# zhangyu2ustc/GCN_fmri_decoding

Hardware: AMD Instinct MI355X
Metric: fMRI-windows/sec (fwd+bwd) 6-layer ChebNet K=5 N≈10k; HBM GB/s vs roofline (higher is better)
Workload: dtype f32; 1 GPU; BASELINE configs[1]: ChebNet K=5 x6 conv (F=32, p=1, b2relu), FC 512-256-22, synthetic N=10000 kNN-8 graph -> M=10466, block_dura=15, batch 64 per GPU; global_batch=64, parallelism=dp1, step=fwd+loss+bwd+allreduce+Adam, batch gathered on device

## Files before the change

gcn_fmri_decoding_amd/_lib.py:

```python
import ctypes as C
import os

_HERE = os.path.dirname(os.path.abspath(__file__))
LIB_PATH = os.environ.get('CHEBGCN_LIB') or os.path.join(_HERE, 'libchebgcn.so')

BIAS_NONE, BIAS_FILTER, BIAS_VERTEX = 0, 1, 2
POOL_MAX, POOL_AVG = 0, 1
KNN_EUCLIDEAN, KNN_COSINE, KNN_CORRELATION, KNN_DOT = 0, 1, 2, 3
KNN_KMAX = 32
MC_SITES = 16
PARCEL_MEAN, PARCEL_SUM = 0, 1


class ChebgcnError(RuntimeError):
    pass


_p = C.c_void_p
_i = C.c_int
_i64 = C.c_int64
_f = C.c_float

SIGNATURES = {
    'chebgcn_version': (_i, []),
# ... 33 lines not shown
    'chebgcn_brelu_pool_bwd_workspace': (C.c_size_t, [_i, _i, _i, _i, _i]),
    'chebgcn_brelu_pool_bwd': (_i, [_p, _p, _p, _p, _p, _i, _i, _i, _i, _i, _i, _i, _p, C.c_size_t, _p]),
    'chebgcn_pool_gather_fwd': (_i, [_p, _p, _p, _p, _i, _i, _i, _i, _i, _i, _p]),
    'chebgcn_pool_scatter_bwd_workspace': (C.c_size_t, [_i, _i, _i, _i, _i]),
    'chebgcn_pool_scatter_bwd': (_i, [_p, _p, _p, _p, _p, _i, _i, _i, _i, _i, _i, _i, _p, C.c_size_t, _p]),
    'chebgcn_contract_bwd_w_workspace': (C.c_size_t, [_i, _i, _i, _i, _i]),
    'chebgcn_contract_bwd_w': (_i, [_p, _p, _p, _p, C.c_size_t, _i, _i, _i, _i, _i, _p]),
    'chebgcn_contract_bwd_x': (_i, [_p, _p, _p, _i, _i, _i, _i, _i, _p]),
    'chebgcn_contract_bwd_x_relu': (_i, [_p, _p, _p, _p, _i, _i, _i, _i, _i, _p]),
    'chebgcn_contract_bwd_w_relu': (_i, [_p, _p, _p, _p, _p, C.c_size_t, _i, _i, _i, _i, _i, _p]),
    'chebgcn_contract_bwd_w_relu_bias_merged': (_i, [_i, _i, _i, _i, _i]),
    'chebgcn_contract_bwd_w_relu_bias': (_i, [_p, _p, _p, _p, _p, _p, C.c_size_t, _i, _i, _i, _i, _i, _p]),
    'chebgcn_contract_fwd_mean_supported': (_i, [_i, _i, _i, _i, _i]),
    'chebgcn_contract_fwd_gated_supported': (_i, [_i, _i, _i, _i, _i]),
    'chebgcn_contract_fwd_gated': (_i, [_p, _p, _p, _p, _i, _i, _i, _i, _i, _p]),
    'chebgcn_contract_fwd_mean': (_i, [_p, _p, _p, _i, _p, _p, _i, _i, _i, _i, _i, _p]),
    'chebgcn_contract_bwd_w_relu_mean': (_i, [_p, _p, _p, _p, _p, C.c_size_t, _i, _i, _i, _i, _i, _p]),
    'chebgcn_contract_bwd_x_relu_mean': (_i, [_p, _p, _p, _p, _i, _i, _i, _i, _i, _p]),
    'chebgcn_bias_grad_relu_mean': (_i, [_p, _p, _p, _i, _i, _i, _i, _p, C.c_size_t, _p]),
    'chebgcn_relu_grad_mean': (_i, [_p, _p, _p, _p, _i, _i, _i, _i, _p, C.c_size_t, _p]),
    'chebgcn_fused_layer_supported': (_i, [_p, _i, _i, _i, _i]),
    'chebgcn_fused_layer_workspace': (C.c_size_t, [_p, _i, _i, _i, _i]),
    'chebgcn_fused_layer_fwd': (_i, [_p, _p, _p, _p, _i, _p, _p, _p, _p, C.c_size_t, _i, _i, _i, _i, _i, _p]),
    'chebgcn_fused_layer_bwd_x': (_i, [_p, _p, _p, _p, _p, _i, _i, _i, _i, _p]),
    'chebgcn_perm_data': (_i, [_p, _p, _p, _p, _i, _i, _i, _i, _p]),
    'chebgcn_to_plane': (_i, [_p, _p, _i, _i, _i, _p]),
    'chebgcn_from_plane': (_i, [_p, _p, _i, _i, _i, _p]),
    'chebgcn_feature_mean_fwd': (_i, [_p, _p, _i, _i, _i, _p]),
    'chebgcn_feature_mean_bwd': (_i, [_p, _p, _i, _i, _i, _p]),
    'chebgcn_fc_fwd_supported': (_i, [_i, _i, _i]),
    'chebgcn_fc_fwd_workspace': (C.c_size_t, [_i, _i, _i]),
    'chebgcn_fc_fwd': (_i, [_p, _i64, _p, _p, _p, _p, C.c_size_t, _i, _i, _i, _i, _p]),
    'chebgcn_fc_bwd': (_i, [_p, _i64, _p, _p, _p, _p, _p, _p, _i64, _i, _i, _i, _p]),
    'chebgcn_planes_to_rows': (_i, [_p, _p, _p, _i, _i, _i, _i64, _p]),
    'chebgcn_rows_to_planes': (_i, [_p, _p, _p, _i, _i, _i, _i64, _p]),
    'chebgcn_adam_step': (_i, [_p, _p, _p, _p, _i64, _f, _f, _f, _f, _f, _f, _p]),
    'chebgcn_adam_step_dev': (_i, [_p, _p, _p, _p, _i64, _p, _f, _f, _f, _f, _f, _p]),
    'chebgcn_metis_one_level_f32': (_i, [_i64, _p, _p, _p, _p, _p, _i64, _p]),
    'chebgcn_metis_one_level_f32p': (_i, [_i64, _p, _p, _p, _p, _p, _i64, _p]),
    'chebgcn_metis_one_level_f64': (_i, [_i64, _p, _p, _p, _p, _p, _i64, _p]),
    'chebgcn_compute_perm_level': (_i, [_p, _i64, _p, _i64, _p]),
    'chebgcn_bank_order': (_i, [_i, _p, _p, _i, _p, _p]),
    'chebgcn_spectral_transform': (_i, [_p, _p, _p, _i, _i, _i, _p]),
    'chebgcn_spectral_mix_fwd': (_i, [_p, _p, _p, _i, _i, _i, _i, _p]),
    'chebgcn_spectral_mix_bwd_x': (_i, [_p, _p, _p, _i, _i, _i, _i, _p]),
    'chebgcn_spectral_mix_bwd_w': (_i, [_p, _p, _p, _i, _i, _i, _i, _p]),
    'chebgcn_spectral_spline_expand': (_i, [_p, _p, _p, _i, _i, _i, _p]),
    'chebgcn_spectral_spline_expand_bwd': (_i, [_p, _p, _p, _i, _i, _i, _p]),
    'chebgcn_saliency_supported': (_i, [_i]),
    'chebgcn_saliency_seed': (_i, [_p, _p, _i, _i, _i, _p, _p, _i, _i, _p]),
    'chebgcn_saliency_path': (_i, [_p, _p, _p, _p, _p, _i, _i, _i, _i, _i, _i, _p]),
    'chebgcn_saliency_reduce': (_i, [_p, _p, _p, _p, _p, _i, _i, _i, _i, _i, _i, _p, _p, _i, _p, _p]),
    'chebgcn_occlusion_supported': (_i, [_i]),
    'chebgcn_occlusion_rows': (_i, [_p, _p, _p, _p, _p, _i64, _i, _i, _i, _i, _i, _i, _p]),
    'chebgcn_occlusion_score': (_i, [_p, _i64, _i, _i, _i, _i, _p, _i, _p, _p, _p]),
    'chebgcn_occlusion_class_sums': (_i, [_p, _p, _i, _i, _i, _p, _p]),
    'chebgcn_shapley_supported': (_i, [_i]),
    'chebgcn_shapley_rows': (_i, [_p, _p, _p, _p, _p, _p, _i64, _i, _i, _i, _i, _i, _i, _i, _p]),
    'chebgcn_shapley_score': (_i, [_p, _i64, _i, _i, _i, _i, _i, _p, _i, _p, _p]),
    'chebgcn_shapley_reduce': (_i, [_p, _p, _i, _i, _i, _p, _p]),
    'chebgcn_gradcam_weights': (_i, [_p, _i, _i, _i, _p, _p]),
    'chebgcn_gradcam_map': (_i, [_p, _p, _p, _p, _i, _i, _i, _i, _i, _p, _i64, _p]),
    'chebgcn_gather_windows': (_i, [_p, _i64, _p, _p, _p, _p, _p, _i, _i, _i, _p]),
    'chebgcn_gather_windows_mix': (_i, [_p, _i64, _p, _p, _i, _p, _p, _p, _p, _i, _i, _i, _p]),
    'chebgcn_window_stats_workspace': (C.c_size_t, [_i64, _i, _i]),
    'chebgcn_window_stats': (_i, [_p, _i64, _p, _i64, _p, _p, _p, _p, _i, _i, _p, C.c_size_t, _p]),
# ... 59 lines not shown
```

gcn_fmri_decoding_amd/csrc/head.hip:

```cpp
#include <hip/hip_runtime.h>
#include "../../include/chebgcn.h"
#include "status.h"
#include "contract_common.h"
#include "aug_draw.h"

namespace chebgcn {

constexpr int FC_WAVES = 8;
constexpr int FC_CHUNK = 32;
constexpr int FC_U = 2;

__global__ void __launch_bounds__(FC_WAVES * 64)
fc_fwd_kernel(const float* __restrict__ x, long long ldx, const float* __restrict__ W, const float* __restrict__ bias,
              float* __restrict__ y, float* __restrict__ part_out, int B, int I, int O, int relu, int cps) {
    __shared__ float part[FC_WAVES][32][33];
    const int lane = threadIdx.x & 63, wave = threadIdx.x >> 6;
    const int c = lane & 31, h = lane >> 5;
    const int bx = blockIdx.x, by = blockIdx.y, bz = blockIdx.z;
    const int o0 = bx * 32, b0 = by * 32;
    const int brow = min(b0 + c, B - 1), ocol = min(o0 + c, O - 1);
    const float* xr = x + (size_t)brow * ldx;
    const float* wc = W + ocol;
    const int nchunks = (I + FC_CHUNK - 1) / FC_CHUNK;
    const int q_lo = bz * cps, q_hi = min(q_lo + cps, nchunks);
    f32x16 acc;
#pragma unroll
    for (int j = 0; j < 16; ++j) acc[j] = 0.f;
    for (int q0 = q_lo + wave; q0 < q_hi; q0 += FC_WAVES * FC_U) {
        f32x4 av[FC_U][4];
        float bv[FC_U][4][4];
#pragma unroll
        for (int u = 0; u < FC_U; ++u) {
            const int q = q0 + FC_WAVES * u;
            const int k = (q < q_hi ? FC_CHUNK * q : 0) + 16 * h;
#pragma unroll
            for (int t = 0; t < 4; ++t) {
                av[u][t] = *reinterpret_cast<const f32x4*>(xr + (k + 4 * t + 3 < ldx ? k + 4 * t : 0));
// ... 328 lines not shown
        }
        const float et = expf(row[t] - m);
        acc += et > 1e-30f ? log1pf(so / et) : logf(s) - (row[t] - m);
        const float inv = invB / s;
        for (int c = 0; c < C; ++c) drow[c] = c == t ? -so * inv : expf(row[c] - m) * inv;
    }
    part[threadIdx.x] = acc;
    __syncthreads();
    for (int d = 128; d > 0; d >>= 1) {
        if ((int)threadIdx.x < d) part[threadIdx.x] += part[threadIdx.x + d];
        __syncthreads();
    }
    if (threadIdx.x == 0) *loss = part[0] * invB;
}
}

using namespace chebgcn;

static int fc_splits(int B, int I, int O) {
    const int tiles = ((O + 31) / 32) * ((B + 31) / 32);
    int s = 512 / tiles;
    const int by_len = (I + 511) / 512;
    if (s > by_len) s = by_len;
    return s < 1 ? 1 : s;
}

extern "C" int chebgcn_fc_fwd_supported(int B, int I, int O) {
    return B > 0 && I > 0 && O > 0 && I <= (1 << 20) && (long long)B * O <= (1 << 20);
}

extern "C" size_t chebgcn_fc_fwd_workspace(int B, int I, int O) {
    if (!chebgcn_fc_fwd_supported(B, I, O)) return 0;
    const int S = fc_splits(B, I, O);
    return S > 1 ? (size_t)S * B * O * sizeof(float) : 0;
}

extern "C" int chebgcn_fc_fwd(const float* x, int64_t ldx, const float* W, const float* bias, float* y, void* workspace,
                              size_t workspace_bytes, int B, int I, int O, int relu, chebgcn_stream stream_) {
    hipStream_t stream = (hipStream_t)stream_;
    CG_REQUIRE(x && W && y && B > 0 && I > 0 && O > 0 && ldx >= I, "fc_fwd: bad argument");
    if (!chebgcn_fc_fwd_supported(B, I, O) || (ldx & 3) || ((uintptr_t)x & 15))
        return CHEBGCN_EUNSUPPORTED;
    const int S = fc_splits(B, I, O);
    const int nchunks = (I + FC_CHUNK - 1) / FC_CHUNK, cps = (nchunks + S - 1) / S;
    CG_REQUIRE(S == 1 || (workspace && workspace_bytes >= chebgcn_fc_fwd_workspace(B, I, O)), "fc_fwd: workspace too small");
    dim3 grid((O + 31) / 32, (B + 31) / 32, S);
    note_dispatch(S > 1 ? "fc_fwd_kernel<split>" : "fc_fwd_kernel");
    if (S > 1) note_dispatch_more("fc_fwd_reduce_kernel");
    hipLaunchKernelGGL(fc_fwd_kernel, grid, dim3(FC_WAVES * 64), 0, stream, x, (long long)ldx, W, bias, y,
                       S > 1 ? (float*)workspace : nullptr, B, I, O, relu, cps);
    if (S > 1)
        hipLaunchKernelGGL(fc_fwd_reduce_kernel, dim3((B * O + 255) / 256), dim3(256), 0, stream, (const float*)workspace, bias,
                           y, B * O, O, S, relu);
    CG_HIP(hipGetLastError());
    return CHEBGCN_OK;
}

static int fc_dropout_splits(int S, int B, int I, int O) {
    const long long tiles = (long long)S * ((O + 31) / 32) * ((B + 31) / 32);
    long long s = 512 / tiles;
    const int by_len = (I + 511) / 512;
    if (s > by_len) s = by_len;
    return s < 1 ? 1 : (int)s;
}

extern "C" int chebgcn_fc_fwd_dropout_supported(int S, int B, int I, int O) {
    return S > 0 && S <= 32768 && B > 0 && I > 0 && O > 0 && I <= (1 << 20) && (long long)S * B * O <= (1 << 20);
}

extern "C" size_t chebgcn_fc_fwd_dropout_workspace(int S, int B, int I, int O) {
    if (!chebgcn_fc_fwd_dropout_supported(S, B, I, O)) return 0;
    const int ns = fc_dropout_splits(S, B, I, O);
    return ns > 1 ? (size_t)ns * S * B * O * sizeof(float) : 0;
}

// ... 5 lines not shown
    CG_REQUIRE(x && W && y && win && S > 0 && B > 0 && I > 0 && O > 0 && ldx >= I, "fc_fwd_dropout: bad argument");
    CG_REQUIRE(sample_stride == 0 || sample_stride >= (int64_t)(B - 1) * ldx + I,
               "fc_fwd_dropout: a sample stride of %lld elements is neither 0 nor a whole [B][ldx] matrix", (long long)sample_stride);
    CG_REQUIRE(s0 >= 0 && layer >= 0 && layer < CHEBGCN_MC_SITES, "fc_fwd_dropout: bad sample number %d or dropout site %d", s0,
               layer);
    CG_REQUIRE(inv_keep >= 1.f && inv_keep < __builtin_inff(), "fc_fwd_dropout: inv_keep = 1 / keep must be a finite number >= 1");
    if (!chebgcn_fc_fwd_dropout_supported(S, B, I, O) || (ldx & 3) || (sample_stride & 3) || ((uintptr_t)x & 15))
        return CHEBGCN_EUNSUPPORTED;
    const int ns = fc_dropout_splits(S, B, I, O);
    const int nchunks = (I + FC_CHUNK - 1) / FC_CHUNK, cps = (nchunks + ns - 1) / ns;
    CG_REQUIRE(ns == 1 || (workspace && workspace_bytes >= chebgcn_fc_fwd_dropout_workspace(S, B, I, O)),
               "fc_fwd_dropout: workspace too small");
    dim3 grid((O + 31) / 32, (B + 31) / 32, S * ns);
    if (sample_stride == 0)
        note_dispatch(ns > 1 ? "fc_fwd_dropout_kernel<shared, split>" : "fc_fwd_dropout_kernel<shared>");
    else
        note_dispatch(ns > 1 ? "fc_fwd_dropout_kernel<per_sample, split>" : "fc_fwd_dropout_kernel<per_sample>");
    if (ns > 1) note_dispatch_more("fc_fwd_reduce_kernel");
    hipLaunchKernelGGL(fc_fwd_dropout_kernel, grid, dim3(FC_WAVES * 64), 0, stream, x, (long long)ldx, (long long)sample_stride, W,
                       bias, y, ns > 1 ? (float*)workspace : nullptr, win, S, B, I, O, relu, cps, ns, seed, (uint32_t)s0,
                       (uint32_t)layer, threshold, inv_keep);
    if (ns > 1)
        hipLaunchKernelGGL(fc_fwd_reduce_kernel, dim3((S * B * O + 255) / 256), dim3(256), 0, stream, (const float*)workspace,
                           bias, y, S * B * O, O, ns, relu);
    CG_HIP(hipGetLastError());
    return CHEBGCN_OK;
}

extern "C" int chebgcn_fc_bwd(const float* x, int64_t ldx, const float* W, const float* g, const float* y, float* dW,
                              float* db, float* dx, int64_t lddx, int B, int I, int O, chebgcn_stream stream_) {
    hipStream_t stream = (hipStream_t)stream_;
    CG_REQUIRE(x && W && g && B > 0 && I > 0 && O > 0 && ldx >= I && (!dx || lddx >= I), "fc_bwd: bad argument");
    if (!chebgcn_fc_fwd_supported(B, I, O)) return CHEBGCN_EUNSUPPORTED;
    note_dispatch(dW ? "fc_bwd_w_kernel" : "");
    if (dW) {
        dim3 grid((O + 31) / 32, (I + 31) / 32);
        hipLaunchKernelGGL(fc_bwd_w_kernel, grid, dim3(FC_WAVES * 64), 0, stream, x, (long long)ldx, g, y, dW, db, B, I, O);
    }
    if (dx) {
        dim3 grid((I + 31) / 32, (B + 31) / 32);
        const bool vec = (O & 3) == 0 && ((uintptr_t)g & 15) == 0 && ((uintptr_t)W & 15) == 0 && (!y || ((uintptr_t)y & 15) == 0);
        note_dispatch_more(vec ? "fc_bwd_x_kernel<true>" : "fc_bwd_x_kernel<false>");
        if (vec)
            hipLaunchKernelGGL(fc_bwd_x_kernel<true>, grid, dim3(FC_WAVES * 64), 0, stream, g, y, W, dx, (long long)lddx, B, I, O);
        else
            hipLaunchKernelGGL(fc_bwd_x_kernel<false>, grid, dim3(FC_WAVES * 64), 0, stream, g, y, W, dx, (long long)lddx, B, I, O);
    }
    CG_HIP(hipGetLastError());
    return CHEBGCN_OK;
}

static int planes_rows(bool to_rows, const float* src, float* dst, const int32_t* order, int B, int M, int F, int64_t ldr,
                       hipStream_t stream) {
    CG_REQUIRE(src && dst && B > 0 && B <= 65535 && M > 0 && F > 0 && ldr >= (int64_t)M * F,
               to_rows ? "planes_to_rows: bad argument" : "rows_to_planes: bad argument");
    const int Mp = plane_stride(M);
    dim3 grid(((to_rows ? M : Mp) + FLAT_V - 1) / FLAT_V, B);
    note_dispatch(to_rows ? "planes_rows_kernel<to_rows>" : "planes_rows_kernel<to_planes>");
    if (to_rows)
        hipLaunchKernelGGL(planes_rows_kernel<true>, grid, dim3(256), 0, stream, src, dst, order, M, Mp, F, (long long)ldr);
    else
        hipLaunchKernelGGL(planes_rows_kernel<false>, grid, dim3(256), 0, stream, src, dst, order, M, Mp, F, (long long)ldr);
    CG_HIP(hipGetLastError());
    return CHEBGCN_OK;
}

extern "C" int chebgcn_planes_to_rows(const float* planes, float* rows, const int32_t* order, int B, int M, int F, int64_t ldr,
                                      chebgcn_stream stream) {
    return planes_rows(true, planes, rows, order, B, M, F, ldr, (hipStream_t)stream);
}

// ... 21 lines not shown
```

gcn_fmri_decoding_amd/ops.py:

```python
import collections
import ctypes as C
import os
import weakref

import numpy as np
import scipy.sparse as sp
import torch

from . import _lib
from . import graph as _graph
from ._lib import BIAS_FILTER, BIAS_NONE, BIAS_VERTEX, POOL_AVG, POOL_MAX, plane_stride


def _stream():
    return C.c_void_p(torch.cuda.current_stream().cuda_stream)


def _p(t):
    return C.c_void_p(t.data_ptr()) if t is not None else None


class KernelTimers:

    def __init__(self, every=1, by_dispatch=False):
# ... 1083 lines not shown
        dx = dW = None
        if ctx.needs_input_grad[1]:
            dW = spectral_mix_bwd_w(dyh, xh, M)
            if Bs is not None:
                dW = spline_expand(Bs, dW.view(M, -1), transpose=True)
        if ctx.needs_input_grad[0]:
            dx = spectral_transform(spectral_mix(dyh, Wf, M, transpose=True), basis, M, True)
        return dx, dW, None, None, None, None


class FeatureMean(torch.autograd.Function):

    @staticmethod
    def forward(ctx, x, M):
        _require_cuda(x)
        x = x if x.is_contiguous() else x.contiguous()
        B, F, Mp = x.shape
        y = torch.empty((B, M), dtype=torch.float32, device=x.device)
        _lib.check(_lib.lib().chebgcn_feature_mean_fwd(_p(x), _p(y), B, M, F, _stream()), 'feature_mean_fwd')
        ctx.cfg = (B, M, F, Mp)
        return y

    @staticmethod
    def backward(ctx, gy):
        B, M, F, Mp = ctx.cfg
        gy = gy.contiguous()
        dx = torch.empty((B, F, Mp), dtype=torch.float32, device=gy.device)
        _lib.check(_lib.lib().chebgcn_feature_mean_bwd(_p(gy), _p(dx), B, M, F, _stream()), 'feature_mean_bwd')
        return dx, None


FC_BWD_MAX_INNER = int(os.environ.get('CHEBGCN_FC_BWD_MAX_INNER', 4096))
FC_FWD_MAX_INNER = int(os.environ.get('CHEBGCN_FC_FWD_MAX_INNER', 1 << 20))


def fc_forward(x, W, b, relu):
    if not (x.is_cuda and x.dtype == torch.float32 and W.dtype == torch.float32 and x.dim() == 2 and W.is_contiguous()
            and x.stride(1) == 1 and x.stride(0) % 4 == 0 and x.data_ptr() % 16 == 0):
        return None
    B, I = x.shape
    O = W.shape[1]
    L = _lib.lib()
    if I > FC_FWD_MAX_INNER or not L.chebgcn_fc_fwd_supported(B, I, O):
        return None
    y = torch.empty((B, O), dtype=torch.float32, device=x.device)
    nws = L.chebgcn_fc_fwd_workspace(B, I, O)
    ws = _workspace(nws, x.device, 'fc_fwd') if nws else None
    _lib.check(L.chebgcn_fc_fwd(_p(x), x.stride(0), _p(W), _p(b), _p(y), _p(ws), nws, B, I, O, 1 if relu else 0, _stream()),
               'fc_fwd')
    return y


def fc_backward(x, W, g, y, dW, db, need_dx):
    B, I = x.shape
    O = W.shape[1]
    L = _lib.lib()
    if not (x.is_cuda and x.dtype == torch.float32 and x.stride(1) == 1 and W.is_contiguous() and g.is_contiguous()
            and dW.is_contiguous() and db.is_contiguous() and (y is None or y.is_contiguous())
            and I <= FC_BWD_MAX_INNER and L.chebgcn_fc_fwd_supported(B, I, O)):
        return None
    dx = torch.empty((B, I), dtype=torch.float32, device=x.device) if need_dx else None
    _lib.check(L.chebgcn_fc_bwd(_p(x), x.stride(0), _p(W), _p(g), _p(y), _p(dW), _p(db), _p(dx), I, B, I, O, _stream()),
               'fc_bwd')
    return (dx,)


def adam_step_sq_all(p, g, m, v, n_reg, lr_t, sq_partials, beta1=0.9, beta2=0.999, eps=1e-8, grad_scale=1.0, l2=0.0):
    _require_cuda(p, g, m, v, sq_partials)
    n = p.numel()
    if not (g.numel() == m.numel() == v.numel() == n) or n == 0 or not (0 <= n_reg <= n):
        raise ValueError('adam_step_sq_all: size mismatch')
    lib = _lib.lib()
    nparts = lib.chebgcn_adam_partials(n)
    if sq_partials.dtype != torch.float32 or sq_partials.numel() < nparts:
        raise ValueError('adam_step_sq_all: sq_partials needs %d float32' % nparts)
    dev_lr = isinstance(lr_t, torch.Tensor)
    if dev_lr and (lr_t.dtype != torch.float32 or lr_t.numel() != 1 or not lr_t.is_cuda):
        raise ValueError('adam_step_sq_all: a device lr_t must be one float32')
    _lib.check(lib.chebgcn_adam_step_sq_all(_p(p), _p(g), _p(m), _p(v), n, int(n_reg), 0.0 if dev_lr else float(lr_t),
                                            _p(lr_t) if dev_lr else None, float(beta1), float(beta2), float(eps), float(grad_scale),
                                            float(l2), _p(sq_partials), _stream()), 'adam_step_sq_all')
    return nparts


def nadam_step_sq_all(p, g, m, v, n_reg, lr_t, sq_partials, beta1=0.9, beta2=0.999, eps=1e-8, grad_scale=1.0, l2=0.0):
    _require_cuda(p, g, m, v, sq_partials)
    n = p.numel()
    if not (g.numel() == m.numel() == v.numel() == n) or n == 0 or not (0 <= n_reg <= n):
        raise ValueError('nadam_step_sq_all: size mismatch')
    lib = _lib.lib()
    nparts = lib.chebgcn_adam_partials(n)
    if sq_partials.dtype != torch.float32 or sq_partials.numel() < nparts:
# ... 10 lines not shown

def planes_to_rows(planes, M, order=None, ld=None):
    _require_cuda(planes)
    B, F, Mp = planes.shape
    if Mp != plane_stride(M) or not planes.is_contiguous():
        raise ValueError('planes_to_rows: planes of %d vertices expected' % M)
    ld = ld or ((M * F + 3) & ~3)
    rows = torch.empty((B, ld), dtype=torch.float32, device=planes.device)
    _lib.check(_launch('planes_to_rows', 8.0 * B * M * F, 0.0, lambda: _lib.lib().chebgcn_planes_to_rows(
        _p(planes), _p(rows), _p(order), B, M, F, ld, _stream())), 'planes_to_rows')
    return rows


def rows_to_planes(rows, M, F, order=None):
    _require_cuda(rows)
    B, ld = rows.shape
    if ld < M * F or rows.stride(1) != 1 or rows.stride(0) != ld:
        raise ValueError('rows_to_planes: rows of at least %d floats expected' % (M * F))
    planes = torch.empty((B, F, plane_stride(M)), dtype=torch.float32, device=rows.device)
    _lib.check(_launch('rows_to_planes', 8.0 * B * M * F, 0.0, lambda: _lib.lib().chebgcn_rows_to_planes(
        _p(rows), _p(planes), _p(order), B, M, F, ld, _stream())), 'rows_to_planes')
    return planes


class FlatFC(torch.autograd.Function):

    @staticmethod
    def forward(ctx, x, W, b, order, M, relu, gW, gb):
        _require_cuda(x, W, b)
        B, F, Mp = x.shape
        I, O = M * F, W.shape[1]
        if tuple(W.shape) != (I, O) or tuple(b.shape) != (O,):
            raise ValueError('FlatFC: weights [%d, O] and bias [O] expected' % I)
        L = _lib.lib()
        if not L.chebgcn_fc_fwd_supported(B, I, O):
            raise ValueError('FlatFC: %d x %d x %d is outside the range of chebgcn_fc_fwd' % (B, I, O))
        rows = planes_to_rows(x.contiguous(), M, order)
        ld = rows.shape[1]
        Wc, bc = W.detach().contiguous(), b.detach().contiguous()
        y = torch.empty((B, O), dtype=torch.float32, device=x.device)
        nws = L.chebgcn_fc_fwd_workspace(B, I, O)
        ws = _workspace(nws, x.device, 'fc_fwd') if nws else None
        _lib.check(_launch('fc_fwd', 4.0 * (B * I + I * O + B * O), 2.0 * B * I * O, lambda: L.chebgcn_fc_fwd(
            _p(rows), ld, _p(Wc), _p(bc), _p(y), _p(ws), nws, B, I, O, 1 if relu else 0, _stream())), 'fc_fwd')
        ctx.save_for_backward(rows, Wc, y if relu else None)
        ctx.cfg, ctx.order, ctx.bufs = (B, M, F, I, O), order, (gW, gb)
        return y

    @staticmethod
    def backward(ctx, g):
        rows, Wc, y = ctx.saved_tensors
        B, M, F, I, O = ctx.cfg
        gW, gb = ctx.bufs
        g = g.contiguous()
        need_w = ctx.needs_input_grad[1] or ctx.needs_input_grad[2]
        dW = db = drows = None
        if need_w:
            dW = gW if gW is not None else torch.empty((I, O), dtype=torch.float32, device=g.device)
            db = gb if gb is not None else torch.empty((O,), dtype=torch.float32, device=g.device)
            _check_grad_buffer(dW, (I, O), 'dW')
            _check_grad_buffer(db, (O,), 'db')
        if ctx.needs_input_grad[0]:
            drows = torch.empty(rows.shape, dtype=torch.float32, device=g.device)
        ld = rows.shape[1]
        if need_w or drows is not None:
            _lib.check(_launch('fc_bwd', 4.0 * (B * I * (1 + (drows is not None)) + I * O * (1 + need_w) + B * O),
                               2.0 * B * I * O * (need_w + (drows is not None)), lambda: _lib.lib().chebgcn_fc_bwd(
                _p(rows), ld, _p(Wc), _p(g), _p(y), _p(dW), _p(db), _p(drows), ld, B, I, O, _stream())), 'fc_bwd')
        dx = rows_to_planes(drows, M, F, ctx.order) if drows is not None else None
        return (dx, None if gW is not None else dW, None if gb is not None else db, None, None, None, None, None)


def adam_step_sq(p, g, m, v, lr_t, sq_partials, beta1=0.9, beta2=0.999, eps=1e-8, grad_scale=1.0, l2=0.0):
    _require_cuda(p, g, m, v, sq_partials)
    n = p.numel()
    if not (g.numel() == m.numel() == v.numel() == n) or n == 0:
        raise ValueError('adam_step_sq: size mismatch')
    lib = _lib.lib()
    nparts = lib.chebgcn_adam_partials(n)
    if sq_partials.dtype != torch.float32 or sq_partials.numel() < nparts:
        raise ValueError('adam_step_sq: sq_partials needs %d float32' % nparts)
    dev_lr = isinstance(lr_t, torch.Tensor)
    if dev_lr and (lr_t.dtype != torch.float32 or lr_t.numel() != 1 or not lr_t.is_cuda):
        raise ValueError('adam_step_sq: a device lr_t must be one float32')
    _lib.check(lib.chebgcn_adam_step_sq(_p(p), _p(g), _p(m), _p(v), n, 0.0 if dev_lr else float(lr_t), _p(lr_t) if dev_lr else None,
                                        float(beta1), float(beta2), float(eps), float(grad_scale), float(l2), _p(sq_partials),
                                        _stream()), 'adam_step_sq')
    return nparts


def loss_bookkeeping(cross_entropy, sq_partials, nparts, half_reg, ema, corr, decay=0.9):
    _require_cuda(cross_entropy, ema)
    out = torch.empty((), dtype=torch.float32, device=ema.device)
    dev_c = isinstance(corr, torch.Tensor)
    _lib.check(_lib.lib().chebgcn_loss_bookkeeping(_p(cross_entropy), _p(sq_partials) if nparts else None, int(nparts), float(half_reg),
                                                   _p(ema), float(decay), 0.0 if dev_c else float(corr), _p(corr) if dev_c else None,
                                                   None, _p(out), _stream()), 'loss_bookkeeping')
    return out


# ... 4 lines not shown
        raise ValueError('adam_step: size mismatch')
    if isinstance(lr_t, torch.Tensor):
        _require_cuda(lr_t)
        if lr_t.dtype != torch.float32 or lr_t.numel() != 1:
            raise ValueError('adam_step: a device lr_t must be one float32')
        _lib.check(_lib.lib().chebgcn_adam_step_dev(_p(p), _p(g), _p(m), _p(v), n, _p(lr_t), float(beta1), float(beta2),
                                                    float(eps), float(grad_scale), float(l2), _stream()), 'adam_step_dev')
        return
    _lib.check(_lib.lib().chebgcn_adam_step(_p(p), _p(g), _p(m), _p(v), n, float(lr_t), float(beta1), float(beta2),
                                            float(eps), float(grad_scale), float(l2), _stream()), 'adam_step')



SCORES = {'logit': 0, 'logprob': 1}
SALIENCY_METHODS = {'gradient': 0, 'grad_x_input': 1, 'integrated': 2}


def _fc_rows(x):
    B, I = x.shape
    if x.stride(1) == 1 and x.stride(0) % 4 == 0 and x.stride(0) >= I and x.data_ptr() % 16 == 0:
        return x
    buf = torch.empty((B, (I + 3) & ~3), dtype=torch.float32, device=x.device)
    buf[:, :I].copy_(x)
    return buf[:, :I]


class FCInputGrad(torch.autograd.Function):

    @staticmethod
    def forward(ctx, x, W, b, relu):
        _require_cuda(x, W, b)
        B, I = x.shape
        O = W.shape[1]
        L = _lib.lib()
        if not L.chebgcn_fc_fwd_supported(B, I, O):
            raise ValueError('saliency: the FC layer %d x %d x %d is outside the range of chebgcn_fc_fwd' % (B, I, O))
        rows = _fc_rows(x.detach())
        Wc, bc = W.detach().contiguous(), b.detach().contiguous()
        y = torch.empty((B, O), dtype=torch.float32, device=x.device)
        nws = L.chebgcn_fc_fwd_workspace(B, I, O)
        ws = _workspace(nws, x.device, 'fc_fwd') if nws else None
        _lib.check(_launch('fc_fwd', 4.0 * (B * I + I * O + B * O), 2.0 * B * I * O, lambda: L.chebgcn_fc_fwd(
            _p(rows), rows.stride(0), _p(Wc), _p(bc), _p(y), _p(ws), nws, B, I, O, 1 if relu else 0, _stream())), 'fc_fwd')
        ctx.save_for_backward(rows, Wc, y if relu else None)
        return y

    @staticmethod
    def backward(ctx, g):
        rows, Wc, y = ctx.saved_tensors
        B, I = rows.shape
        O = Wc.shape[1]
        g = g.contiguous()
        dx = torch.empty((B, I), dtype=torch.float32, device=g.device)
        _lib.check(_launch('fc_bwd_x', 4.0 * (B * I + I * O + B * O), 2.0 * B * I * O, lambda: _lib.lib().chebgcn_fc_bwd(
            _p(rows), rows.stride(0), _p(Wc), _p(g), _p(y), None, None, _p(dx), I, B, I, O, _stream())), 'fc_bwd_x')
        return dx, None, None, None


def saliency_seed(logits, targets, rep, nvalid, score, cls_out=None, want_grad=True):
    _require_cuda(logits, targets, cls_out)
    z = logits.detach().contiguous()
    B, C = z.shape
    for t, what in ((targets, 'targets'), (cls_out, 'cls_out')):
        if t is not None and (t.dtype != torch.int64 or not t.is_contiguous() or t.numel() < (nvalid + rep - 1) // rep):
            raise ValueError('saliency_seed: %s must be contiguous int64 with a value per window' % what)
    dz = torch.empty_like(z) if want_grad else None
    _lib.check(_launch('saliency_seed', 4.0 * 2 * B * C, 0.0, lambda: _lib.lib().chebgcn_saliency_seed(
        _p(z), _p(targets), int(rep), int(nvalid), SCORES[score], _p(dz), _p(cls_out), B, C, _stream())), 'saliency_seed')
    return dz


def saliency_path(data, order, sample, baseline, R, steps, M):
    _require_cuda(data, order, sample, baseline)
    S, N, F = data.shape
    nw = int(sample.numel())
    out = torch.empty((int(R), F, plane_stride(M)), dtype=torch.float32, device=data.device)
    _lib.check(_launch('saliency_path', 4.0 * F * (nw * N * (1 + (baseline is not None)) + R * plane_stride(M)), 0.0,
                       lambda: _lib.lib().chebgcn_saliency_path(_p(data), _p(order), _p(sample), _p(baseline), _p(out), nw,
                                                                int(steps), int(R), N, int(M), F, _stream())), 'saliency_path')
    return out


def saliency_reduce(dx, data, order, sample, baseline, steps, method, absolute, out, cls=None, acc=None):
    _require_cuda(dx, data, order, sample, baseline, out, cls, acc)
    nw, M, F = out.shape
    if not out.is_contiguous() or dx.shape[1] != F or dx.shape[0] < nw * steps or not dx.is_contiguous():
        raise ValueError('saliency_reduce: shapes of dx %s and out %s do not match' % (tuple(dx.shape), tuple(out.shape)))
# ... 101 lines not shown
    _require_cuda(A, G, order, out)
    A = A.detach()
    G = G.detach()
    A = A if A.is_contiguous() else A.contiguous()
    G = G if G.is_contiguous() else G.contiguous()
    B, F, Mp = A.shape
    if (tuple(G.shape) != (B, F, Mp) or Mp != plane_stride(N) or B < nw or out.dtype != torch.float32
            or not out.is_contiguous() or tuple(out.shape) != (nw, N * P)
            or (order is not None and (order.dtype != torch.int32 or order.numel() != N))):
        raise ValueError('gradcam_map: A and G [>= %d, F, %d], out float32 [%d, %d], order int32 [%d]'
                         % (nw, plane_stride(N), nw, N * P, N))
    L = _lib.lib()
    alpha = None
    if GRADCAM_METHODS[method] == 0:
        alpha = torch.empty((nw, F), dtype=torch.float32, device=A.device)
        _lib.check(_launch('gradcam_weights', 4.0 * nw * F * (N + 1), 0.0, lambda: L.chebgcn_gradcam_weights(
            _p(G), nw, F, N, _p(alpha), _stream())), 'gradcam_weights')
    nbytes = 4.0 * (nw * F * N * (1 + (alpha is None)) + (N if order is not None else 0) + nw * N * P)
    _lib.check(_launch('gradcam_map', nbytes, 2.0 * nw * F * N, lambda: L.chebgcn_gradcam_map(
        _p(A), _p(G) if alpha is None else None, _p(alpha), _p(order), nw, F, N, P, int(bool(relu)), _p(out), N * P,
        _stream())), 'gradcam_map')
    return out



MC_SAMPLES_MAX = 1024
MC_CLASSES_MAX = 64


def fc_forward_native(x, W, b, relu, who):
    _require_cuda(x, W, b)
    B, I = x.shape
    O = W.shape[1]
    L = _lib.lib()
    if not L.chebgcn_fc_fwd_supported(B, I, O):
        raise ValueError('%s: the FC layer %d x %d x %d is outside the range of chebgcn_fc_fwd' % (who, B, I, O))
    rows = _fc_rows(x.detach())
    Wc, bc = W.detach().contiguous(), b.detach().contiguous()
    y = torch.empty((B, O), dtype=torch.float32, device=x.device)
    nws = L.chebgcn_fc_fwd_workspace(B, I, O)
    ws = _workspace(nws, x.device, 'fc_fwd') if nws else None
    _lib.check(_launch('fc_fwd', 4.0 * (B * I + I * O + B * O), 2.0 * B * I * O, lambda: L.chebgcn_fc_fwd(
        _p(rows), rows.stride(0), _p(Wc), _p(bc), _p(y), _p(ws), nws, B, I, O, 1 if relu else 0, _stream())), 'fc_fwd')
    return y


def _fc_sample_rows(x):
    S, B, I = x.shape
    if (x.stride(2) == 1 and x.stride(1) % 4 == 0 and x.stride(1) >= I and x.stride(0) % 4 == 0
            and x.stride(0) >= (B - 1) * x.stride(1) + I and x.data_ptr() % 16 == 0):
        return x
    buf = torch.zeros((S, B, (I + 3) & ~3), dtype=torch.float32, device=x.device)
    buf[:, :, :I].copy_(x)
    return buf[:, :, :I]


def fc_forward_dropout(x, W, b, relu, win, S, s0, layer, seed, threshold, inv_keep):
    _require_cuda(x, W, b, win)
    shared = x.dim() == 2
    rows = _fc_rows(x.detach()) if shared else _fc_sample_rows(x.detach())
    B, I = rows.shape[-2:]
    O = W.shape[1]
    S = int(S)
    if not shared and rows.shape[0] != S:
        raise ValueError('fc_forward_dropout: x holds %d samples, S = %d' % (rows.shape[0], S))
    if win.dtype != torch.int32 or not win.is_contiguous() or win.numel() != B:
        raise ValueError('fc_forward_dropout: win must be a contiguous int32 vector with a window number per row')
# ... 32 lines not shown
```

include/chebgcn.h:

```cpp
#ifndef CHEBGCN_H
#define CHEBGCN_H

#include <stddef.h>
#include <stdint.h>

#ifdef __cplusplus
extern "C" {
#endif

#define CHEBGCN_VERSION 1

enum {
    CHEBGCN_OK = 0,
    CHEBGCN_EINVAL = -1,
    CHEBGCN_EHIP = -2,
    CHEBGCN_ENOMEM = -3,
    CHEBGCN_EUNSUPPORTED = -4
};

enum { CHEBGCN_BIAS_NONE = 0, CHEBGCN_BIAS_FILTER = 1 , CHEBGCN_BIAS_VERTEX = 2  };
enum { CHEBGCN_POOL_MAX = 0, CHEBGCN_POOL_AVG = 1 };

typedef struct chebgcn_graph chebgcn_graph;
typedef void* chebgcn_stream;
// ... 103 lines not shown
                                     int Fin, int K, int Fout, chebgcn_stream stream);
int chebgcn_contract_bwd_x_relu_mean(const float* gmean, const uint8_t* relu_mask, const float* W,
                                     float* gstack, int B, int M, int Fin, int K, int Fout,
                                     chebgcn_stream stream);
int chebgcn_bias_grad_relu_mean(const float* gmean, const uint8_t* relu_mask, float* dbias, int bias_kind,
                                int B, int M, int F, void* workspace, size_t workspace_bytes,
                                chebgcn_stream stream);
int chebgcn_relu_grad_mean(const float* gmean, const uint8_t* relu_mask, float* dy, float* dbias, int bias_kind,
                           int B, int M, int F, void* workspace, size_t workspace_bytes,
                           chebgcn_stream stream);

int chebgcn_fused_layer_supported(const chebgcn_graph* g, int B, int Fin, int K, int Fout);
size_t chebgcn_fused_layer_workspace(const chebgcn_graph* g, int B, int Fin, int K, int Fout);
int chebgcn_fused_layer_fwd(const chebgcn_graph* g, const float* x, const float* W, const float* bias, int bias_kind,
                            float* stack, float* out, uint8_t* relu_mask, void* workspace, size_t workspace_bytes,
                            int B, int Fin, int K, int Fout, int relu, chebgcn_stream stream);
int chebgcn_fused_layer_bwd_x(const chebgcn_graph* g, const float* dout, const uint8_t* relu_mask, const float* W,
                              float* dx, int B, int Fin, int K, int Fout, chebgcn_stream stream);

int chebgcn_perm_data(const float* x, const int32_t* perm, const int32_t* sample, float* out,
                      int S, int N, int M, int F, chebgcn_stream stream);
int chebgcn_to_plane(const float* x_bmf, float* out_plane, int B, int M, int F, chebgcn_stream stream);
int chebgcn_from_plane(const float* x_plane, float* out_bmf, int B, int M, int F, chebgcn_stream stream);

int chebgcn_feature_mean_fwd(const float* x, float* y, int B, int M, int F, chebgcn_stream stream);
int chebgcn_feature_mean_bwd(const float* dy, float* dx, int B, int M, int F, chebgcn_stream stream);

int chebgcn_fc_fwd_supported(int B, int I, int O);
size_t chebgcn_fc_fwd_workspace(int B, int I, int O);
int chebgcn_fc_fwd(const float* x, int64_t ldx, const float* W, const float* bias, float* y, void* workspace,
                   size_t workspace_bytes, int B, int I, int O, int relu, chebgcn_stream stream);
int chebgcn_fc_bwd(const float* x, int64_t ldx, const float* W, const float* g, const float* y, float* dW, float* db,
                   float* dx, int64_t lddx, int B, int I, int O, chebgcn_stream stream);

int chebgcn_planes_to_rows(const float* planes, float* rows, const int32_t* order, int B, int M, int F, int64_t ldr,
                           chebgcn_stream stream);
int chebgcn_rows_to_planes(const float* rows, float* planes, const int32_t* order, int B, int M, int F, int64_t ldr,
                           chebgcn_stream stream);

int chebgcn_set_scalars(float* dst, float v0, float v1, chebgcn_stream stream);

int chebgcn_adam_partials(int64_t n);
int chebgcn_adam_step_sq(float* p, const float* g, float* m, float* v, int64_t n, float lr_t, const float* lr_t_dev,
                         float beta1, float beta2, float eps, float grad_scale, float l2, float* sq_partials,
                         chebgcn_stream stream);
int chebgcn_adam_step_sq_all(float* p, const float* g, float* m, float* v, int64_t n, int64_t n_reg, float lr_t,
                             const float* lr_t_dev, float beta1, float beta2, float eps, float grad_scale, float l2,
                             float* sq_partials, chebgcn_stream stream);
int chebgcn_nadam_step_sq_all(float* p, const float* g, float* m, float* v, int64_t n, int64_t n_reg, float lr_t,
                              const float* lr_t_dev, float beta1, float beta2, float eps, float grad_scale, float l2,
                              float* sq_partials, chebgcn_stream stream);
int chebgcn_loss_bookkeeping(const float* cross_entropy, const float* sq_partials, int nparts, float half_reg, float* ema,
                             float decay, float corr, const float* corr_dev, float* loss_out, float* loss_average_out,
                             chebgcn_stream stream);

int chebgcn_softmax_xent(const float* logits, const void* labels, int labels_int64, float* loss, float* dlogits, int B,
                         int C, chebgcn_stream stream);

int chebgcn_adam_step(float* p, const float* g, float* m, float* v, int64_t n, float lr_t,
                      float beta1, float beta2, float eps, float grad_scale, float l2,
                      chebgcn_stream stream);
int chebgcn_adam_step_dev(float* p, const float* g, float* m, float* v, int64_t n, const float* lr_t_dev,
                          float beta1, float beta2, float eps, float grad_scale, float l2,
                          chebgcn_stream stream);

int chebgcn_metis_one_level_f32(int64_t nnz, const int64_t* rr, const int64_t* cc, const float* vv,
// ... 119 lines not shown
```

Before: 21760 windows/s.

## Add wide-inner FC kernels for the flattened first FC layer fwd and dW

Adds a dedicated path for FC layers with a very large inner dimension and small batch, which is the flattened graph-to-512 layer. The forward kernel covers up to 64 batch rows per block with MFMA, splits the inner dimension across waves with a deep register prefetch, reduces partials in shared memory, and finishes with a split-K reduce kernel. A new dW kernel stages masked gradients in LDS and computes 128-column output tiles. The backward path now uses a native kernel even when the inner size exceeds the old 4096 limit, where it previously fell back. This adds a workspace requirement and more code paths, with an environment switch to turn it off.

```diff
diff --git a/gcn_fmri_decoding_amd/_lib.py b/gcn_fmri_decoding_amd/_lib.py
--- a/gcn_fmri_decoding_amd/_lib.py
+++ b/gcn_fmri_decoding_amd/_lib.py
@@ -89,6 +89,8 @@
     'chebgcn_fc_fwd_workspace': (C.c_size_t, [_i, _i, _i]),
     'chebgcn_fc_fwd': (_i, [_p, _i64, _p, _p, _p, _p, C.c_size_t, _i, _i, _i, _i, _p]),
     'chebgcn_fc_bwd': (_i, [_p, _i64, _p, _p, _p, _p, _p, _p, _i64, _i, _i, _i, _p]),
+    'chebgcn_fc_wide_supported': (_i, [_i, _i, _i]),
+    'chebgcn_fc_wide_enable': (_i, [_i]),
     'chebgcn_planes_to_rows': (_i, [_p, _p, _p, _i, _i, _i, _i64, _p]),
     'chebgcn_rows_to_planes': (_i, [_p, _p, _p, _i, _i, _i, _i64, _p]),
     'chebgcn_adam_step': (_i, [_p, _p, _p, _p, _i64, _f, _f, _f, _f, _f, _f, _p]),
diff --git a/gcn_fmri_decoding_amd/csrc/head.hip b/gcn_fmri_decoding_amd/csrc/head.hip
--- a/gcn_fmri_decoding_amd/csrc/head.hip
+++ b/gcn_fmri_decoding_amd/csrc/head.hip
@@ -3,6 +3,7 @@
 #include "status.h"
 #include "contract_common.h"
 #include "aug_draw.h"
+#include "head_wide.h"
 
 namespace chebgcn {
 
@@ -397,7 +398,7 @@
 extern "C" size_t chebgcn_fc_fwd_workspace(int B, int I, int O) {
     if (!chebgcn_fc_fwd_supported(B, I, O)) return 0;
     const int S = fc_splits(B, I, O);
-    return S > 1 ? (size_t)S * B * O * sizeof(float) : 0;
+    return S > 1 || fc_wide_shape(B, I, O) ? (size_t)S * B * O * sizeof(float) : 0;
 }
 
 extern "C" int chebgcn_fc_fwd(const float* x, int64_t ldx, const float* W, const float* bias, float* y, void* workspace,
@@ -406,6 +407,18 @@
     CG_REQUIRE(x && W && y && B > 0 && I > 0 && O > 0 && ldx >= I, "fc_fwd: bad argument");
     if (!chebgcn_fc_fwd_supported(B, I, O) || (ldx & 3) || ((uintptr_t)x & 15))
         return CHEBGCN_EUNSUPPORTED;
+    if (fc_wide_on(B, I, O)) {
+        int bps = 0;
+        const int Sw = fc_wide_splits(B, I, O, fc_splits(B, I, O), &bps);
+        CG_REQUIRE(workspace && workspace_bytes >= (size_t)Sw * B * O * sizeof(float), "fc_fwd: workspace too small");
+        note_dispatch("fc_fwd_kernel<wide>");
+        note_dispatch_more("fc_fwd_reduce_kernel");
+        fc_fwd_wide_launch(x, (long long)ldx, W, (float*)workspace, B, I, O, Sw, bps, stream);
+        hipLaunchKernelGGL(fc_fwd_reduce_kernel, dim3((B * O + 255) / 256), dim3(256), 0, stream, (const float*)workspace, bias,
+                           y, B * O, O, Sw, relu);
+        CG_HIP(hipGetLastError());
+        return CHEBGCN_OK;
+    }
     const int S = fc_splits(B, I, O);
     const int nchunks = (I + FC_CHUNK - 1) / FC_CHUNK, cps = (nchunks + S - 1) / S;
     CG_REQUIRE(S == 1 || (workspace && workspace_bytes >= chebgcn_fc_fwd_workspace(B, I, O)), "fc_fwd: workspace too small");
@@ -477,11 +490,16 @@
     hipStream_t stream = (hipStream_t)stream_;
     CG_REQUIRE(x && W && g && B > 0 && I > 0 && O > 0 && ldx >= I && (!dx || lddx >= I), "fc_bwd: bad argument");
     if (!chebgcn_fc_fwd_supported(B, I, O)) return CHEBGCN_EUNSUPPORTED;
-    note_dispatch(dW ? "fc_bwd_w_kernel" : "");
-    if (dW) {
+    const bool wide = fc_wide_on(B, I, O);
+    const char* wname = "";
+    if (dW && wide) {
+        wname = fc_bwd_w_wide_launch(x, (long long)ldx, g, y, dW, db, B, I, O, stream);
+    } else if (dW) {
+        wname = "fc_bwd_w_kernel";
         dim3 grid((O + 31) / 32, (I + 31) / 32);
         hipLaunchKernelGGL(fc_bwd_w_kernel, grid, dim3(FC_WAVES * 64), 0, stream, x, (long long)ldx, g, y, dW, db, B, I, O);
     }
+    note_dispatch(wname);
     if (dx) {
         dim3 grid((I + 31) / 32, (B + 31) / 32);
         const bool vec = (O & 3) == 0 && ((uintptr_t)g & 15) == 0 && ((uintptr_t)W & 15) == 0 && (!y || ((uintptr_t)y & 15) == 0);
diff --git a/gcn_fmri_decoding_amd/csrc/head_wide.h b/gcn_fmri_decoding_amd/csrc/head_wide.h
--- /dev/null
+++ b/gcn_fmri_decoding_amd/csrc/head_wide.h
@@ -0,0 +1,22 @@
+#pragma once
+#include <hip/hip_runtime.h>
+#include <stddef.h>
+#include <stdint.h>
+
+namespace chebgcn {
+
+constexpr int FC_WIDE_MAX_BATCH = 64;
+constexpr int FC_WIDE_MIN_INNER = 8192;
+constexpr int FC_WIDE_MIN_WEIGHTS = 1 << 20;
+
+bool fc_wide_shape(int B, int I, int O);
+bool fc_wide_on(int B, int I, int O);
+
+int fc_wide_splits(int B, int I, int O, int max_splits, int* bps);
+
+void fc_fwd_wide_launch(const float* x, long long ldx, const float* W, float* part, int B, int I, int O, int S, int bps,
+                        hipStream_t stream);
+const char* fc_bwd_w_wide_launch(const float* x, long long ldx, const float* g, const float* y, float* dW, float* db, int B, int I,
+                                 int O, hipStream_t stream);
+
+}
diff --git a/gcn_fmri_decoding_amd/csrc/head_wide.hip b/gcn_fmri_decoding_amd/csrc/head_wide.hip
--- /dev/null
+++ b/gcn_fmri_decoding_amd/csrc/head_wide.hip
@@ -0,0 +1,236 @@
+#include <hip/hip_runtime.h>
+#include <stdlib.h>
+#include <atomic>
+#include "../../include/chebgcn.h"
+#include "status.h"
+#include "contract_common.h"
+#include "head_wide.h"
+
+namespace chebgcn {
+
+constexpr int FW_WAVES = 8;
+constexpr int FW_KB = 8;
+constexpr int FW_D = 6;
+
+#define MFMA(a, b, c) __builtin_amdgcn_mfma_f32_32x32x2f32((a), (b), (c), 0, 0, 0)
+
+template <bool TWO>
+__global__ void __launch_bounds__(FW_WAVES * 64)
+fc_fwd_wide_kernel(const float* __restrict__ x, long long ldx, const float* __restrict__ W, float* __restrict__ part_out, int B,
+                   int I, int O, int bps) {
+    __shared__ float slab[FW_WAVES / 2][64][32];
+    const int lane = threadIdx.x & 63, wave = threadIdx.x >> 6;
+    const int c = lane & 31, h = lane >> 5;
+    const int z = blockIdx.x, o0 = blockIdx.y * 32;
+    const int nblk = (I + FW_KB - 1) / FW_KB;
+    const int q_lo = z * bps, q_hi = min(q_lo + bps, nblk);
+    const int bpw = (q_hi - q_lo + FW_WAVES - 1) / FW_WAVES;
+    const int w_lo = q_lo + wave * bpw, w_hi = min(w_lo + bpw, q_hi);
+    const float* x0 = x + (size_t)min(c, B - 1) * ldx;
+    const float* x1 = x + (size_t)min(32 + c, B - 1) * ldx;
+    const float* wc = W + min(o0 + c, O - 1);
+    f32x16 acc[2];
+#pragma unroll
+    for (int r = 0; r < 2; ++r)
+#pragma unroll
+        for (int j = 0; j < 16; ++j) acc[r][j] = 0.f;
+    f32x4 xa[FW_D][2];
+    float wv[FW_D][4];
+#define FW_LOAD(u, q)                                                                                          \
+    if ((q) < w_hi) {                                                                                          \
+        const int k_ = FW_KB * (q) + 4 * h;                                                                    \
+        xa[u][0] = *reinterpret_cast<const f32x4*>(x0 + (k_ + 3 < ldx ? k_ : 0));                              \
+        if (TWO) xa[u][1] = *reinterpret_cast<const f32x4*>(x1 + (k_ + 3 < ldx ? k_ : 0));                     \
+        _Pragma("unroll") for (int t = 0; t < 4; ++t) wv[u][t] = wc[(size_t)(k_ + t < I ? k_ + t : 0) * O];   \
+    }
+#pragma unroll
+    for (int u = 0; u < FW_D; ++u) {
+        xa[u][0] = xa[u][1] = f32x4{0.f, 0.f, 0.f, 0.f};
+#pragma unroll
+        for (int t = 0; t < 4; ++t) wv[u][t] = 0.f;
+        FW_LOAD(u, w_lo + u)
+    }
+    for (int q0 = w_lo; q0 < w_hi; q0 += FW_D) {
+#pragma unroll
+        for (int u = 0; u < FW_D; ++u) {
+            const int q = q0 + u;
+            const int k = FW_KB * q + 4 * h;
+#pragma unroll
+            for (int t = 0; t < 4; ++t) {
+                const bool ok = q < w_hi && k + t < I;
+                const float b = ok ? wv[u][t] : 0.f;
+                acc[0] = MFMA(ok ? xa[u][0][t] : 0.f, b, acc[0]);
+                if (TWO) acc[1] = MFMA(ok ? xa[u][1][t] : 0.f, b, acc[1]);
+            }
+            FW_LOAD(u, q + FW_D)
+        }
+    }
+#undef FW_LOAD
+    constexpr int HALF = FW_WAVES / 2;
+    if (wave >= HALF) {
+#pragma unroll
+        for (int r = 0; r < 2; ++r)
+#pragma unroll
+            for (int j = 0; j < 16; ++j) slab[wave - HALF][32 * r + acc_row(j, h)][c] = acc[r][j];
+    }
+    __syncthreads();
+    if (wave < HALF) {
+#pragma unroll
+        for (int r = 0; r < 2; ++r)
+#pragma unroll
+            for (int j = 0; j < 16; ++j) slab[wave][32 * r + acc_row(j, h)][c] += acc[r][j];
+    }
+    __syncthreads();
+    const int rows = min(B, TWO ? 64 : 32);
+    for (int e = threadIdx.x; e < rows * 32; e += FW_WAVES * 64) {
+        const int r = e >> 5, cc = e & 31;
+        float s = slab[0][r][cc];
+#pragma unroll
+        for (int w = 1; w < HALF; ++w) s += slab[w][r][cc];
+        if (o0 + cc < O) part_out[((size_t)z * B + r) * O + o0 + cc] = s;
+    }
+}
+
+constexpr int BW_WAVES = 4;
+constexpr int BW_COLS = 128;
+
+template <bool VEC>
+__global__ void __launch_bounds__(BW_WAVES * 64)
+fc_bwd_w_wide_kernel(const float* __restrict__ x, long long ldx, const float* __restrict__ g, const float* __restrict__ y,
+                     float* __restrict__ dW, float* __restrict__ db, int B, int I, int O) {
+    __shared__ f32x4 gm[64][BW_COLS / 4];
+    const int lane = threadIdx.x & 63, wave = threadIdx.x >> 6;
+    const int c = lane & 31, h = lane >> 5;
+    const int o0 = blockIdx.x * BW_COLS, i0 = (blockIdx.y * BW_WAVES + wave) * 32;
+    const int icol = min(i0 + c, I - 1);
+    const int nch = (B + 7) >> 3;
+    float xa[8][4];
+#pragma unroll
+    for (int q = 0; q < 8; ++q)
+#pragma unroll
+        for (int j = 0; j < 4; ++j) {
+            const int b = 8 * q + 4 * h + j;
+            xa[q][j] = (q < nch && b < B) ? x[(size_t)b * ldx + icol] : 0.f;
+        }
+    for (int e = threadIdx.x; e < 64 * (BW_COLS / 4); e += BW_WAVES * 64) {
+        const int b = e / (BW_COLS / 4), cq = e % (BW_COLS / 4);
+        const int col = o0 + 4 * cq;
+        f32x4 v = {0.f, 0.f, 0.f, 0.f};
+        if (b < B) {
+            if (VEC) {
+                const size_t at = (size_t)b * O + min(col, O - 4);
+                v = *reinterpret_cast<const f32x4*>(g + at);
+                if (y) {
+                    const f32x4 yv = *reinterpret_cast<const f32x4*>(y + at);
+#pragma unroll
+                    for (int jj = 0; jj < 4; ++jj) v[jj] = yv[jj] > 0.f ? v[jj] : 0.f;
+                }
+            } else {
+#pragma unroll
+                for (int jj = 0; jj < 4; ++jj) {
+                    const size_t at = (size_t)b * O + min(col + jj, O - 1);
+                    v[jj] = (!y || y[at] > 0.f) ? g[at] : 0.f;
+                }
+            }
+        }
+        gm[b][cq] = v;
+    }
+    __syncthreads();
+    if (i0 >= I) return;
+    f32x16 acc[4];
+#pragma unroll
+    for (int jj = 0; jj < 4; ++jj)
+#pragma unroll
+        for (int j = 0; j < 16; ++j) acc[jj][j] = 0.f;
+    f32x4 bsum = {0.f, 0.f, 0.f, 0.f};
+#pragma unroll
+    for (int q = 0; q < 8; ++q) {
+        if (q < nch) {
+#pragma unroll
+            for (int j = 0; j < 4; ++j) {
+                const f32x4 m = gm[8 * q + 4 * h + j][c];
+                bsum += m;
+#pragma unroll
+                for (int jj = 0; jj < 4; ++jj) acc[jj] = MFMA(xa[q][j], m[jj], acc[jj]);
+            }
+        }
+    }
+    const int col = o0 + 4 * c;
+#pragma unroll
+    for (int j = 0; j < 16; ++j) {
+        const int row = i0 + acc_row(j, h);
+        if (row >= I) continue;
+        float* out = dW + (size_t)row * O;
+        if (VEC) {
+            if (col < O) *reinterpret_cast<f32x4*>(out + col) = f32x4{acc[0][j], acc[1][j], acc[2][j], acc[3][j]};
+        } else {
+#pragma unroll
+            for (int jj = 0; jj < 4; ++jj)
+                if (col + jj < O) out[col + jj] = acc[jj][j];
+        }
+    }
+    if (db && blockIdx.y == 0 && wave == 0) {
+#pragma unroll
+        for (int jj = 0; jj < 4; ++jj) {
+            const float other = __shfl_xor(bsum[jj], 32);
+            if (h == 0 && col + jj < O) db[col + jj] = bsum[jj] + other;
+        }
+    }
+}
+
+#undef MFMA
+
+static std::atomic<int>& wide_switch() {
+    static std::atomic<int> on([] {
+        const char* e = getenv("CHEBGCN_FC_WIDE");
+        return (e && e[0] == '0' && !e[1]) ? 0 : 1;
+    }());
+    return on;
+}
+
+bool fc_wide_shape(int B, int I, int O) {
+    return B > 0 && B <= FC_WIDE_MAX_BATCH && O > 0 && I >= FC_WIDE_MIN_INNER && I <= (1 << 20) &&
+           (long long)I * O >= FC_WIDE_MIN_WEIGHTS && (long long)B * O <= (1 << 20);
+}
+
+bool fc_wide_on(int B, int I, int O) { return wide_switch().load(std::memory_order_relaxed) != 0 && fc_wide_shape(B, I, O); }
+
+int fc_wide_splits(int B, int I, int O, int max_splits, int* bps_out) {
+    const int groups = (O + 31) / 32;
+    const int nblk = (I + FW_KB - 1) / FW_KB;
+    int s = 256 / groups;
+    if (s > max_splits) s = max_splits;
+    if (s > nblk / FW_WAVES) s = nblk / FW_WAVES;
+    if (s < 1) s = 1;
+    const int bps = (nblk + s - 1) / s;
+    if (bps_out) *bps_out = bps;
+    return (nblk + bps - 1) / bps;
+}
+
+void fc_fwd_wide_launch(const float* x, long long ldx, const float* W, float* part, int B, int I, int O, int S, int bps,
+                        hipStream_t stream) {
+    const dim3 grid(S, (O + 31) / 32), block(FW_WAVES * 64);
+    if (B > 32)
+        hipLaunchKernelGGL(fc_fwd_wide_kernel<true>, grid, block, 0, stream, x, ldx, W, part, B, I, O, bps);
+    else
+        hipLaunchKernelGGL(fc_fwd_wide_kernel<false>, grid, block, 0, stream, x, ldx, W, part, B, I, O, bps);
+}
+
+const char* fc_bwd_w_wide_launch(const float* x, long long ldx, const float* g, const float* y, float* dW, float* db, int B, int I,
+                                 int O, hipStream_t stream) {
+    const dim3 grid((O + BW_COLS - 1) / BW_COLS, (I + 32 * BW_WAVES - 1) / (32 * BW_WAVES)), block(BW_WAVES * 64);
+    const bool vec = (O & 3) == 0 && (((uintptr_t)g | (uintptr_t)dW | (uintptr_t)y) & 15) == 0;
+    if (vec)
+        hipLaunchKernelGGL(fc_bwd_w_wide_kernel<true>, grid, block, 0, stream, x, ldx, g, y, dW, db, B, I, O);
+    else
+        hipLaunchKernelGGL(fc_bwd_w_wide_kernel<false>, grid, block, 0, stream, x, ldx, g, y, dW, db, B, I, O);
+    return vec ? "fc_bwd_w_kernel<wide>" : "fc_bwd_w_kernel<wide>[scalar]";
+}
+
+}
+
+using namespace chebgcn;
+
+extern "C" int chebgcn_fc_wide_supported(int B, int I, int O) { return fc_wide_shape(B, I, O) ? 1 : 0; }
+
+extern "C" int chebgcn_fc_wide_enable(int on) { return wide_switch().exchange(on ? 1 : 0); }
diff --git a/gcn_fmri_decoding_amd/ops.py b/gcn_fmri_decoding_amd/ops.py
--- a/gcn_fmri_decoding_amd/ops.py
+++ b/gcn_fmri_decoding_amd/ops.py
@@ -1139,6 +1139,24 @@
 
 FC_BWD_MAX_INNER = int(os.environ.get('CHEBGCN_FC_BWD_MAX_INNER', 4096))
 FC_FWD_MAX_INNER = int(os.environ.get('CHEBGCN_FC_FWD_MAX_INNER', 1 << 20))
+fc_wide = os.environ.get('CHEBGCN_FC_WIDE', '1') != '0'
+_fc_wide_sent = None
+
+
+def _fc_lib():
+    global _fc_wide_sent
+    L = _lib.lib()
+    if _fc_wide_sent != bool(fc_wide):
+        _fc_wide_sent = bool(fc_wide)
+        L.chebgcn_fc_wide_enable(1 if _fc_wide_sent else 0)
+    return L
+
+
+def set_fc_wide(on):
+    global fc_wide
+    was, fc_wide = bool(fc_wide), bool(on)
+    _fc_lib()
+    return was
 
 
 def fc_forward(x, W, b, relu):
@@ -1147,7 +1165,7 @@
         return None
     B, I = x.shape
     O = W.shape[1]
-    L = _lib.lib()
+    L = _fc_lib()
     if I > FC_FWD_MAX_INNER or not L.chebgcn_fc_fwd_supported(B, I, O):
         return None
     y = torch.empty((B, O), dtype=torch.float32, device=x.device)
@@ -1161,10 +1179,11 @@
 def fc_backward(x, W, g, y, dW, db, need_dx):
     B, I = x.shape
     O = W.shape[1]
-    L = _lib.lib()
+    L = _fc_lib()
+    wide = fc_wide and L.chebgcn_fc_wide_supported(B, I, O)
     if not (x.is_cuda and x.dtype == torch.float32 and x.stride(1) == 1 and W.is_contiguous() and g.is_contiguous()
             and dW.is_contiguous() and db.is_contiguous() and (y is None or y.is_contiguous())
-            and I <= FC_BWD_MAX_INNER and L.chebgcn_fc_fwd_supported(B, I, O)):
+            and (I <= FC_BWD_MAX_INNER or wide) and L.chebgcn_fc_fwd_supported(B, I, O)):
         return None
     dx = torch.empty((B, I), dtype=torch.float32, device=x.device) if need_dx else None
     _lib.check(L.chebgcn_fc_bwd(_p(x), x.stride(0), _p(W), _p(g), _p(y), _p(dW), _p(db), _p(dx), I, B, I, O, _stream()),
@@ -1241,7 +1260,7 @@
         I, O = M * F, W.shape[1]
         if tuple(W.shape) != (I, O) or tuple(b.shape) != (O,):
             raise ValueError('FlatFC: weights [%d, O] and bias [O] expected' % I)
-        L = _lib.lib()
+        L = _fc_lib()
         if not L.chebgcn_fc_fwd_supported(B, I, O):
             raise ValueError('FlatFC: %d x %d x %d is outside the range of chebgcn_fc_fwd' % (B, I, O))
         rows = planes_to_rows(x.contiguous(), M, order)
@@ -1274,7 +1293,7 @@
         ld = rows.shape[1]
         if need_w or drows is not None:
             _lib.check(_launch('fc_bwd', 4.0 * (B * I * (1 + (drows is not None)) + I * O * (1 + need_w) + B * O),
-                               2.0 * B * I * O * (need_w + (drows is not None)), lambda: _lib.lib().chebgcn_fc_bwd(
+                               2.0 * B * I * O * (need_w + (drows is not None)), lambda: _fc_lib().chebgcn_fc_bwd(
                 _p(rows), ld, _p(Wc), _p(g), _p(y), _p(dW), _p(db), _p(drows), ld, B, I, O, _stream())), 'fc_bwd')
         dx = rows_to_planes(drows, M, F, ctx.order) if drows is not None else None
         return (dx, None if gW is not None else dW, None if gb is not None else db, None, None, None, None, None)
@@ -1345,7 +1364,7 @@
         _require_cuda(x, W, b)
         B, I = x.shape
         O = W.shape[1]
-        L = _lib.lib()
+        L = _fc_lib()
         if not L.chebgcn_fc_fwd_supported(B, I, O):
             raise ValueError('saliency: the FC layer %d x %d x %d is outside the range of chebgcn_fc_fwd' % (B, I, O))
         rows = _fc_rows(x.detach())
@@ -1365,7 +1384,7 @@
         O = Wc.shape[1]
         g = g.contiguous()
         dx = torch.empty((B, I), dtype=torch.float32, device=g.device)
-        _lib.check(_launch('fc_bwd_x', 4.0 * (B * I + I * O + B * O), 2.0 * B * I * O, lambda: _lib.lib().chebgcn_fc_bwd(
+        _lib.check(_launch('fc_bwd_x', 4.0 * (B * I + I * O + B * O), 2.0 * B * I * O, lambda: _fc_lib().chebgcn_fc_bwd(
             _p(rows), rows.stride(0), _p(Wc), _p(g), _p(y), None, None, _p(dx), I, B, I, O, _stream())), 'fc_bwd_x')
         return dx, None, None, None
 
@@ -1533,7 +1552,7 @@
     _require_cuda(x, W, b)
     B, I = x.shape
     O = W.shape[1]
-    L = _lib.lib()
+    L = _fc_lib()
     if not L.chebgcn_fc_fwd_supported(B, I, O):
         raise ValueError('%s: the FC layer %d x %d x %d is outside the range of chebgcn_fc_fwd' % (who, B, I, O))
     rows = _fc_rows(x.detach())
diff --git a/include/chebgcn.h b/include/chebgcn.h
--- a/include/chebgcn.h
+++ b/include/chebgcn.h
@@ -159,6 +159,8 @@
                    size_t workspace_bytes, int B, int I, int O, int relu, chebgcn_stream stream);
 int chebgcn_fc_bwd(const float* x, int64_t ldx, const float* W, const float* g, const float* y, float* dW, float* db,
                    float* dx, int64_t lddx, int B, int I, int O, chebgcn_stream stream);
+int chebgcn_fc_wide_supported(int B, int I, int O);
+int chebgcn_fc_wide_enable(int on);
 
 int chebgcn_planes_to_rows(const float* planes, float* rows, const int32_t* order, int B, int M, int F, int64_t ldr,
                            chebgcn_stream stream);
```

After: 21810 windows/s, median of 6. No clear change (+0.2%).
